# thunlp/OpenMatch

Measured on NVIDIA H100. Metric: queries/sec top-1000 over 8.8M x 768 corpus, higher is better.
Workload: dtype f16

## Files before the change

openmatch_b200/csrc/ptx.cuh:

```cuda
#pragma once
#include <cuda_runtime.h>
#include <cuda_bf16.h>
#include <stdint.h>

#ifndef OM_WAIT_TIMEOUT_CYCLES
#define OM_WAIT_TIMEOUT_CYCLES (1000000000ll)
#endif

namespace om {

static __device__ unsigned int om_dev_fault;

__device__ __forceinline__ uint32_t smem_u32(const void* p) {
  return static_cast<uint32_t>(__cvta_generic_to_shared(p));
}

__device__ __forceinline__ void mbar_init(uint64_t* bar, uint32_t count) {
  asm volatile("mbarrier.init.shared::cta.b64 [%0], %1;" ::"r"(smem_u32(bar)), "r"(count) : "memory");
}
__device__ __forceinline__ void fence_barrier_init() {
  asm volatile("fence.mbarrier_init.release.cluster;" ::: "memory");
}
__device__ __forceinline__ void fence_proxy_async_smem() {
  asm volatile("fence.proxy.async.shared::cta;" ::: "memory");
}
__device__ __forceinline__ void fence_proxy_async_global() {
  asm volatile("fence.proxy.async.global;" ::: "memory");
}
__device__ __forceinline__ void mbar_arrive_expect_tx(uint64_t* bar, uint32_t bytes) {
  asm volatile("mbarrier.arrive.expect_tx.shared::cta.b64 _, [%0], %1;" ::"r"(smem_u32(bar)), "r"(bytes)
               : "memory");
}
__device__ __forceinline__ void mbar_arrive(uint64_t* bar) {
  asm volatile("mbarrier.arrive.shared::cta.b64 _, [%0];" ::"r"(smem_u32(bar)) : "memory");
}
__device__ __forceinline__ bool mbar_try_wait(uint64_t* bar, uint32_t parity) {
  uint32_t done;
  asm volatile(
      "{\n\t"
      ".reg .pred P;\n\t"
      "mbarrier.try_wait.parity.shared::cta.b64 P, [%1], %2;\n\t"
      "selp.u32 %0, 1, 0, P;\n\t"
      "}\n"
      : "=r"(done)
      : "r"(smem_u32(bar)), "r"(parity)
      : "memory");
  return done != 0;
}
static __device__ __noinline__ void mbar_wait_slow(uint64_t* bar, uint32_t parity, uint32_t site) {
  const long long t0 = clock64();
  uint32_t spins = 0;
  while (!mbar_try_wait(bar, parity)) {
    if ((++spins & 1023u) != 0) continue;
    if (*reinterpret_cast<volatile unsigned int*>(&om_dev_fault) != 0u) return;
    if (clock64() - t0 > OM_WAIT_TIMEOUT_CYCLES) {
      atomicCAS(&om_dev_fault, 0u, (site << 16) | (blockIdx.x & 0xffffu) | 0x80000000u);
      return;
    }
  }
}
__device__ __forceinline__ void mbar_wait(uint64_t* bar, uint32_t parity, uint32_t site) {
  if (mbar_try_wait(bar, parity)) return;
  if (mbar_try_wait(bar, parity)) return;
  mbar_wait_slow(bar, parity, site);
}
__device__ __forceinline__ void mbar_wait_warp(uint64_t* bar, uint32_t parity, uint32_t site) {
  if ((threadIdx.x & 31u) == 0) {
    if (!mbar_try_wait(bar, parity)) {
      const long long t0 = clock64();
      uint32_t spins = 0;
      while (!mbar_try_wait(bar, parity)) {
        __nanosleep(64);
        if ((++spins & 1023u) != 0) continue;
        if (*reinterpret_cast<volatile unsigned int*>(&om_dev_fault) != 0u) break;
        if (clock64() - t0 > OM_WAIT_TIMEOUT_CYCLES) {
          atomicCAS(&om_dev_fault, 0u, (site << 16) | (blockIdx.x & 0xffffu) | 0x80000000u);
          break;
        }
      }
    }
  }
  __syncwarp();
}
static inline unsigned int read_clear_dev_fault() {
  unsigned int v = 0, z = 0;
  if (cudaMemcpyFromSymbol(&v, om_dev_fault, sizeof(v)) != cudaSuccess) return 0xffffffffu;
  if (v) cudaMemcpyToSymbol(om_dev_fault, &z, sizeof(z));
  return v;
}

__device__ __forceinline__ void tma_prefetch_desc(const void* tmap) {
  asm volatile("prefetch.tensormap [%0];" ::"l"(reinterpret_cast<uint64_t>(tmap)) : "memory");
}
__device__ __forceinline__ void tma_load_2d(void* smem_dst, const void* tmap, uint64_t* bar, int32_t c0,
                                            int32_t c1) {
  asm volatile(
      "cp.async.bulk.tensor.2d.shared::cluster.global.tile.mbarrier::complete_tx::bytes"
      " [%0], [%1, {%3, %4}], [%2];"
      ::"r"(smem_u32(smem_dst)), "l"(reinterpret_cast<uint64_t>(tmap)), "r"(smem_u32(bar)), "r"(c0), "r"(c1)
      : "memory");
}
__device__ __forceinline__ void tma_prefetch_l2_2d(const void* tmap, int32_t c0, int32_t c1) {
  asm volatile("cp.async.bulk.prefetch.tensor.2d.L2.global.tile [%0, {%1, %2}];" ::"l"(reinterpret_cast<uint64_t>(tmap)),
               "r"(c0), "r"(c1)
               : "memory");
}
__device__ __forceinline__ void tma_store_2d(const void* tmap, const void* smem_src, int32_t c0, int32_t c1) {
  asm volatile("cp.async.bulk.tensor.2d.global.shared::cta.tile.bulk_group [%0, {%2, %3}], [%1];" ::"l"(
                   reinterpret_cast<uint64_t>(tmap)),
               "r"(smem_u32(smem_src)), "r"(c0), "r"(c1)
               : "memory");
}
__device__ __forceinline__ void bulk_commit_group() { asm volatile("cp.async.bulk.commit_group;" ::: "memory"); }
__device__ __forceinline__ void bulk_wait_group_read0() { asm volatile("cp.async.bulk.wait_group.read 0;" ::: "memory"); }
__device__ __forceinline__ void bulk_wait_group0() { asm volatile("cp.async.bulk.wait_group 0;" ::: "memory"); }

__device__ __forceinline__ void tma_load_2d_multicast(void* smem_dst, const void* tmap, uint64_t* bar, int32_t c0,
                                                      int32_t c1, uint16_t cta_mask) {
  asm volatile(
      "cp.async.bulk.tensor.2d.shared::cluster.global.tile.mbarrier::complete_tx::bytes.multicast::cluster"
      " [%0], [%1, {%3, %4}], [%2], %5;"
      ::"r"(smem_u32(smem_dst)), "l"(reinterpret_cast<uint64_t>(tmap)), "r"(smem_u32(bar)), "r"(c0), "r"(c1),
      "h"(cta_mask)
      : "memory");
}

__device__ __forceinline__ uint32_t cluster_ctarank() {
  uint32_t r;
  asm volatile("mov.u32 %0, %%cluster_ctarank;" : "=r"(r));
  return r;
}
__device__ __forceinline__ uint32_t cluster_id_x() {
  uint32_t r;
  asm volatile("mov.u32 %0, %%clusterid.x;" : "=r"(r));
  return r;
}
__device__ __forceinline__ uint32_t cluster_count_x() {
  uint32_t r;
  asm volatile("mov.u32 %0, %%nclusterid.x;" : "=r"(r));
  return r;
}
__device__ __forceinline__ void cluster_sync_all() {
  asm volatile("barrier.cluster.arrive.release.aligned;\n\tbarrier.cluster.wait.acquire.aligned;" ::: "memory");
}
__device__ __forceinline__ void mbar_arrive_remote(uint64_t* bar, uint32_t rank) {
  asm volatile(
      "{\n\t.reg .b32 ra;\n\t"
      "mapa.shared::cluster.u32 ra, %0, %1;\n\t"
      "mbarrier.arrive.shared::cluster.b64 _, [ra];\n\t}\n"
      ::"r"(smem_u32(bar)), "r"(rank)
      : "memory");
}

__device__ __forceinline__ void wgmma_fence() { asm volatile("wgmma.fence.sync.aligned;" ::: "memory"); }
__device__ __forceinline__ void wgmma_commit() { asm volatile("wgmma.commit_group.sync.aligned;" ::: "memory"); }
template <int N>
__device__ __forceinline__ void wgmma_wait() {
  asm volatile("wgmma.wait_group.sync.aligned %0;" ::"n"(N) : "memory");
}
template <int R>
__device__ __forceinline__ void wgmma_fence_regs(float (&d)[R]) {
#pragma unroll
  for (int i = 0; i < R; ++i) asm volatile("" : "+f"(d[i])::"memory");
}

__host__ __device__ constexpr uint64_t wgmma_desc_base(uint32_t lbo_bytes, uint32_t sbo_bytes) {
  return (static_cast<uint64_t>((lbo_bytes >> 4) & 0x3fffu) << 16) |
         (static_cast<uint64_t>((sbo_bytes >> 4) & 0x3fffu) << 32) | (1ull << 62);
}
__device__ __forceinline__ uint64_t wgmma_desc(uint32_t smem_addr, uint64_t base) {
  return base | static_cast<uint64_t>((smem_addr & 0x3ffffu) >> 4);
}
constexpr uint64_t kDescKMajorSW128 = wgmma_desc_base(16, 1024);

template <int TA, int TB>
__device__ __forceinline__ void wgmma_m64n128k16_bf16(float (&d)[64], uint64_t a_desc, uint64_t b_desc, uint32_t accumulate) {
  asm volatile(
      "{\n\t.reg .pred p;\n\tsetp.ne.b32 p, %66, 0;\n\t"
      "wgmma.mma_async.sync.aligned.m64n128k16.f32.bf16.bf16 {%0, %1, %2, %3, %4, %5, %6, %7, %8, %9, %10, %11, %12, %13, %14, %15, %16, %17, %18, %19, %20, %21, %22, %23, %24, %25, %26, %27, %28, %29, %30, %31, %32, %33, %34, %35, %36, %37, %38, %39, %40, %41, %42, %43, %44, %45, %46, %47, %48, %49, %50, %51, %52, %53, %54, %55, %56, %57, %58, %59, %60, %61, %62, %63}, %64, %65, p, 1, 1, %67, %68;\n\t}\n"
      : "+f"(d[0]), "+f"(d[1]), "+f"(d[2]), "+f"(d[3]), "+f"(d[4]), "+f"(d[5]), "+f"(d[6]), "+f"(d[7]), "+f"(d[8]), "+f"(d[9]), "+f"(d[10]), "+f"(d[11]), "+f"(d[12]), "+f"(d[13]), "+f"(d[14]), "+f"(d[15]), "+f"(d[16]), "+f"(d[17]), "+f"(d[18]), "+f"(d[19]), "+f"(d[20]), "+f"(d[21]), "+f"(d[22]), "+f"(d[23]), "+f"(d[24]), "+f"(d[25]), "+f"(d[26]), "+f"(d[27]), "+f"(d[28]), "+f"(d[29]), "+f"(d[30]), "+f"(d[31]), "+f"(d[32]), "+f"(d[33]), "+f"(d[34]), "+f"(d[35]), "+f"(d[36]), "+f"(d[37]), "+f"(d[38]), "+f"(d[39]), "+f"(d[40]), "+f"(d[41]), "+f"(d[42]), "+f"(d[43]), "+f"(d[44]), "+f"(d[45]), "+f"(d[46]), "+f"(d[47]), "+f"(d[48]), "+f"(d[49]), "+f"(d[50]), "+f"(d[51]), "+f"(d[52]), "+f"(d[53]), "+f"(d[54]), "+f"(d[55]), "+f"(d[56]), "+f"(d[57]), "+f"(d[58]), "+f"(d[59]), "+f"(d[60]), "+f"(d[61]), "+f"(d[62]), "+f"(d[63])
      : "l"(a_desc), "l"(b_desc), "r"(accumulate), "n"(TA), "n"(TB));
}
template <int TA, int TB>
__device__ __forceinline__ void wgmma_m64n128k16_f16(float (&d)[64], uint64_t a_desc, uint64_t b_desc, uint32_t accumulate) {
  asm volatile(
      "{\n\t.reg .pred p;\n\tsetp.ne.b32 p, %66, 0;\n\t"
      "wgmma.mma_async.sync.aligned.m64n128k16.f32.f16.f16 {%0, %1, %2, %3, %4, %5, %6, %7, %8, %9, %10, %11, %12, %13, %14, %15, %16, %17, %18, %19, %20, %21, %22, %23, %24, %25, %26, %27, %28, %29, %30, %31, %32, %33, %34, %35, %36, %37, %38, %39, %40, %41, %42, %43, %44, %45, %46, %47, %48, %49, %50, %51, %52, %53, %54, %55, %56, %57, %58, %59, %60, %61, %62, %63}, %64, %65, p, 1, 1, %67, %68;\n\t}\n"
      : "+f"(d[0]), "+f"(d[1]), "+f"(d[2]), "+f"(d[3]), "+f"(d[4]), "+f"(d[5]), "+f"(d[6]), "+f"(d[7]), "+f"(d[8]), "+f"(d[9]), "+f"(d[10]), "+f"(d[11]), "+f"(d[12]), "+f"(d[13]), "+f"(d[14]), "+f"(d[15]), "+f"(d[16]), "+f"(d[17]), "+f"(d[18]), "+f"(d[19]), "+f"(d[20]), "+f"(d[21]), "+f"(d[22]), "+f"(d[23]), "+f"(d[24]), "+f"(d[25]), "+f"(d[26]), "+f"(d[27]), "+f"(d[28]), "+f"(d[29]), "+f"(d[30]), "+f"(d[31]), "+f"(d[32]), "+f"(d[33]), "+f"(d[34]), "+f"(d[35]), "+f"(d[36]), "+f"(d[37]), "+f"(d[38]), "+f"(d[39]), "+f"(d[40]), "+f"(d[41]), "+f"(d[42]), "+f"(d[43]), "+f"(d[44]), "+f"(d[45]), "+f"(d[46]), "+f"(d[47]), "+f"(d[48]), "+f"(d[49]), "+f"(d[50]), "+f"(d[51]), "+f"(d[52]), "+f"(d[53]), "+f"(d[54]), "+f"(d[55]), "+f"(d[56]), "+f"(d[57]), "+f"(d[58]), "+f"(d[59]), "+f"(d[60]), "+f"(d[61]), "+f"(d[62]), "+f"(d[63])
      : "l"(a_desc), "l"(b_desc), "r"(accumulate), "n"(TA), "n"(TB));
}
template <int TA, int TB>
__device__ __forceinline__ void wgmma_m64n256k16_f16(float (&d)[128], uint64_t a_desc, uint64_t b_desc, uint32_t accumulate) {
  asm volatile(
      "{\n\t.reg .pred p;\n\tsetp.ne.b32 p, %130, 0;\n\t"
      "wgmma.mma_async.sync.aligned.m64n256k16.f32.f16.f16 {%0, %1, %2, %3, %4, %5, %6, %7, %8, %9, %10, %11, %12, %13, %14, %15, %16, %17, %18, %19, %20, %21, %22, %23, %24, %25, %26, %27, %28, %29, %30, %31, %32, %33, %34, %35, %36, %37, %38, %39, %40, %41, %42, %43, %44, %45, %46, %47, %48, %49, %50, %51, %52, %53, %54, %55, %56, %57, %58, %59, %60, %61, %62, %63, %64, %65, %66, %67, %68, %69, %70, %71, %72, %73, %74, %75, %76, %77, %78, %79, %80, %81, %82, %83, %84, %85, %86, %87, %88, %89, %90, %91, %92, %93, %94, %95, %96, %97, %98, %99, %100, %101, %102, %103, %104, %105, %106, %107, %108, %109, %110, %111, %112, %113, %114, %115, %116, %117, %118, %119, %120, %121, %122, %123, %124, %125, %126, %127}, %128, %129, p, 1, 1, %131, %132;\n\t}\n"
      : "+f"(d[0]), "+f"(d[1]), "+f"(d[2]), "+f"(d[3]), "+f"(d[4]), "+f"(d[5]), "+f"(d[6]), "+f"(d[7]), "+f"(d[8]), "+f"(d[9]), "+f"(d[10]), "+f"(d[11]), "+f"(d[12]), "+f"(d[13]), "+f"(d[14]), "+f"(d[15]), "+f"(d[16]), "+f"(d[17]), "+f"(d[18]), "+f"(d[19]), "+f"(d[20]), "+f"(d[21]), "+f"(d[22]), "+f"(d[23]), "+f"(d[24]), "+f"(d[25]), "+f"(d[26]), "+f"(d[27]), "+f"(d[28]), "+f"(d[29]), "+f"(d[30]), "+f"(d[31]), "+f"(d[32]), "+f"(d[33]), "+f"(d[34]), "+f"(d[35]), "+f"(d[36]), "+f"(d[37]), "+f"(d[38]), "+f"(d[39]), "+f"(d[40]), "+f"(d[41]), "+f"(d[42]), "+f"(d[43]), "+f"(d[44]), "+f"(d[45]), "+f"(d[46]), "+f"(d[47]), "+f"(d[48]), "+f"(d[49]), "+f"(d[50]), "+f"(d[51]), "+f"(d[52]), "+f"(d[53]), "+f"(d[54]), "+f"(d[55]), "+f"(d[56]), "+f"(d[57]), "+f"(d[58]), "+f"(d[59]), "+f"(d[60]), "+f"(d[61]), "+f"(d[62]), "+f"(d[63]), "+f"(d[64]), "+f"(d[65]), "+f"(d[66]), "+f"(d[67]), "+f"(d[68]), "+f"(d[69]), "+f"(d[70]), "+f"(d[71]), "+f"(d[72]), "+f"(d[73]), "+f"(d[74]), "+f"(d[75]), "+f"(d[76]), "+f"(d[77]), "+f"(d[78]), "+f"(d[79]), "+f"(d[80]), "+f"(d[81]), "+f"(d[82]), "+f"(d[83]), "+f"(d[84]), "+f"(d[85]), "+f"(d[86]), "+f"(d[87]), "+f"(d[88]), "+f"(d[89]), "+f"(d[90]), "+f"(d[91]), "+f"(d[92]), "+f"(d[93]), "+f"(d[94]), "+f"(d[95]), "+f"(d[96]), "+f"(d[97]), "+f"(d[98]), "+f"(d[99]), "+f"(d[100]), "+f"(d[101]), "+f"(d[102]), "+f"(d[103]), "+f"(d[104]), "+f"(d[105]), "+f"(d[106]), "+f"(d[107]), "+f"(d[108]), "+f"(d[109]), "+f"(d[110]), "+f"(d[111]), "+f"(d[112]), "+f"(d[113]), "+f"(d[114]), "+f"(d[115]), "+f"(d[116]), "+f"(d[117]), "+f"(d[118]), "+f"(d[119]), "+f"(d[120]), "+f"(d[121]), "+f"(d[122]), "+f"(d[123]), "+f"(d[124]), "+f"(d[125]), "+f"(d[126]), "+f"(d[127])
      : "l"(a_desc), "l"(b_desc), "r"(accumulate), "n"(TA), "n"(TB));
}

template <int N>
__device__ __forceinline__ void setmaxnreg_dec() {
  asm volatile("setmaxnreg.dec.sync.aligned.u32 %0;" ::"n"(N));
}
template <int N>
__device__ __forceinline__ void setmaxnreg_inc() {
  asm volatile("setmaxnreg.inc.sync.aligned.u32 %0;" ::"n"(N));
}
__device__ __forceinline__ void wgmma_m64n64k16_bf16_rs(float (&d)[32], const uint32_t (&a)[4], uint64_t b_desc, uint32_t accumulate) {
  asm volatile(
      "{\n\t.reg .pred p;\n\tsetp.ne.b32 p, %37, 0;\n\t"
      "wgmma.mma_async.sync.aligned.m64n64k16.f32.bf16.bf16 {%0, %1, %2, %3, %4, %5, %6, %7, %8, %9, %10, %11, %12, %13, %14, %15, %16, %17, %18, %19, %20, %21, %22, %23, %24, %25, %26, %27, %28, %29, %30, %31}, {%32, %33, %34, %35}, %36, p, 1, 1, 0;\n\t}\n"
      : "+f"(d[0]), "+f"(d[1]), "+f"(d[2]), "+f"(d[3]), "+f"(d[4]), "+f"(d[5]), "+f"(d[6]), "+f"(d[7]), "+f"(d[8]), "+f"(d[9]), "+f"(d[10]), "+f"(d[11]), "+f"(d[12]), "+f"(d[13]), "+f"(d[14]), "+f"(d[15]), "+f"(d[16]), "+f"(d[17]), "+f"(d[18]), "+f"(d[19]), "+f"(d[20]), "+f"(d[21]), "+f"(d[22]), "+f"(d[23]), "+f"(d[24]), "+f"(d[25]), "+f"(d[26]), "+f"(d[27]), "+f"(d[28]), "+f"(d[29]), "+f"(d[30]), "+f"(d[31])
      : "r"(a[0]), "r"(a[1]), "r"(a[2]), "r"(a[3]), "l"(b_desc), "r"(accumulate));
}
__device__ __forceinline__ void wgmma_m64n32k16_bf16_rs(float (&d)[16], const uint32_t (&a)[4], uint64_t b_desc, uint32_t accumulate) {
  asm volatile(
      "{\n\t.reg .pred p;\n\tsetp.ne.b32 p, %21, 0;\n\t"
      "wgmma.mma_async.sync.aligned.m64n32k16.f32.bf16.bf16 {%0, %1, %2, %3, %4, %5, %6, %7, %8, %9, %10, %11, %12, %13, %14, %15}, {%16, %17, %18, %19}, %20, p, 1, 1, 0;\n\t}\n"
      : "+f"(d[0]), "+f"(d[1]), "+f"(d[2]), "+f"(d[3]), "+f"(d[4]), "+f"(d[5]), "+f"(d[6]), "+f"(d[7]), "+f"(d[8]), "+f"(d[9]), "+f"(d[10]), "+f"(d[11]), "+f"(d[12]), "+f"(d[13]), "+f"(d[14]), "+f"(d[15])
      : "r"(a[0]), "r"(a[1]), "r"(a[2]), "r"(a[3]), "l"(b_desc), "r"(accumulate));
}

__device__ __forceinline__ uint32_t pack_bf16x2(float lo, float hi) {
  __nv_bfloat162 v = __floats2bfloat162_rn(lo, hi);
  return *reinterpret_cast<uint32_t*>(&v);
}
__device__ __forceinline__ float2 fma2(float2 a, float2 b, float2 c) { return make_float2(fmaf(a.x, b.x, c.x), fmaf(a.y, b.y, c.y)); }
__device__ __forceinline__ float2 mul2(float2 a, float2 b) { return make_float2(__fmul_rn(a.x, b.x), __fmul_rn(a.y, b.y)); }
__device__ __forceinline__ float2 splat2(float x) { return make_float2(x, x); }

__device__ __forceinline__ void named_bar_sync(uint32_t id, uint32_t nthreads) {
  asm volatile("bar.sync %0, %1;" ::"r"(id), "r"(nthreads) : "memory");
}

}
```

openmatch_b200/csrc/ring.cuh:

```cuda
#pragma once
#include "ptx.cuh"

namespace om {

template <int STAGES>
struct Ring {
  uint32_t stage = 0, phase = 0;
  __device__ __forceinline__ void advance() {
    if (++stage == STAGES) {
      stage = 0;
      phase ^= 1u;
    }
  }
};

__device__ __forceinline__ void ring_init(uint64_t* full, uint64_t* empty, int stages, uint32_t empty_arrivals) {
  for (int i = 0; i < stages; ++i) {
    mbar_init(&full[i], 1);
    mbar_init(&empty[i], empty_arrivals);
  }
}

template <int STAGES>
__device__ __forceinline__ void ring_wait_free(uint64_t* empty, const Ring<STAGES>& r, uint32_t site) {
  mbar_wait(&empty[r.stage], r.phase ^ 1u, site);
}

template <int STAGES>
__device__ __forceinline__ uint64_t* ring_acquire_tx(uint64_t* full, uint64_t* empty, const Ring<STAGES>& r,
                                                     uint32_t bytes, uint32_t site) {
  ring_wait_free(empty, r, site);
  mbar_arrive_expect_tx(&full[r.stage], bytes);
  return &full[r.stage];
}

template <int STAGES, class Issue, class Release>
__device__ __forceinline__ void ring_consume(uint64_t* full, Ring<STAGES>& r, int kb_begin, int kb_end, uint32_t site,
                                             Issue&& issue, Release&& release) {
  uint32_t prev_stage = 0;
  for (int kb = kb_begin; kb < kb_end; ++kb) {
    mbar_wait_warp(&full[r.stage], r.phase, site);
    wgmma_fence();
    issue(r.stage, kb != kb_begin ? 1u : 0u);
    wgmma_commit();
    if (kb != kb_begin) {
      wgmma_wait<1>();
      release(prev_stage);
    }
    prev_stage = r.stage;
    r.advance();
  }
  wgmma_wait<0>();
  if (kb_end > kb_begin) release(prev_stage);
}

}
```

openmatch_b200/csrc/scan_gemm.cuh:

```cuda
#pragma once
#include <cuda_fp16.h>

#include "scan_epilogue.cuh"

namespace om {

constexpr int kScanBlockN = 256;
constexpr int kScanStages = 3;
constexpr int kScanABytes = kBlockM * kBlockK * 2;
constexpr int kScanBBytes = kScanBlockN * kBlockK * 2;
constexpr int kScanStageBytes = kScanABytes + kScanBBytes;
constexpr int kScanConsumers = 256;
constexpr int kScanStash = 4;
constexpr int kScanStashOffset = kScanStages * kScanStageBytes;
constexpr int kScanStashBytes = 2 * 2 * kScanStash * kScanConsumers * 8;
constexpr int kScanBarOffset = kScanStashOffset + kScanStashBytes;
constexpr int kScanSmemBytes = kScanBarOffset + 2 * kScanStages * 8 + 1024;
static_assert(kScanSmemBytes <= 232448, "scan ring + stash exceed the 227 KB of shared memory an H100 block may use");

template <int H>
__device__ __forceinline__ float scan_pick(const float (&acc)[128], int i) {
  float a[32], b[16], c[8], d[4], e[2];
#pragma unroll
  for (int j = 0; j < 32; ++j) a[j] = (i & 1) ? acc[4 * j + 2 * H + 1] : acc[4 * j + 2 * H];
#pragma unroll
  for (int j = 0; j < 16; ++j) b[j] = (i & 2) ? a[2 * j + 1] : a[2 * j];
#pragma unroll
  for (int j = 0; j < 8; ++j) c[j] = (i & 4) ? b[2 * j + 1] : b[2 * j];
#pragma unroll
  for (int j = 0; j < 4; ++j) d[j] = (i & 8) ? c[2 * j + 1] : c[2 * j];
#pragma unroll
  for (int j = 0; j < 2; ++j) e[j] = (i & 16) ? d[2 * j + 1] : d[2 * j];
  return (i & 32) ? e[1] : e[0];
}

template <int H>
__device__ __forceinline__ int scan_filter_row(const float (&acc)[128], float t, int row, int lim, int q4, int col0,
                                               unsigned long long* stash, unsigned long long* cand, int* count,
                                               int* overflow, int C, uint32_t row_base) {
  float mx = acc[2 * H];
#pragma unroll
  for (int j = 0; j < 32; ++j) mx = fmaxf(mx, fmaxf(acc[4 * j + 2 * H], acc[4 * j + 2 * H + 1]));
  if (!(mx > t)) return 0;
  uint32_t lo = 0, hi = 0;
#pragma unroll
  for (int i = 0; i < 32; ++i) {
    lo |= (acc[4 * (i >> 1) + 2 * H + (i & 1)] > t ? 1u : 0u) << i;
    hi |= (acc[4 * (16 + (i >> 1)) + 2 * H + (i & 1)] > t ? 1u : 0u) << i;
  }
  unsigned long long mask = (static_cast<unsigned long long>(hi) << 32) | lo;
  if (lim < kScanBlockN) {
#pragma unroll 1
    for (int i = 0; i < 64; ++i)
      if (8 * (i >> 1) + 2 * q4 + (i & 1) >= lim) mask &= ~(1ull << i);
  }
  const int n = __popcll(mask);
  int pos = 0;
  if (n > kScanStash) {
    pos = atomicAdd(count + row, n - kScanStash);
    if (pos + (n - kScanStash) > C) *overflow = 1;
  }
  unsigned long long* mine = cand + static_cast<size_t>(row) * C;
  int idx = 0;
#pragma unroll 1
  while (mask) {
    const int i = __ffsll(static_cast<long long>(mask)) - 1;
    mask &= mask - 1;
    const unsigned long long key =
        make_key(scan_pick<H>(acc, i), row_base + static_cast<uint32_t>(col0 + 8 * (i >> 1) + 2 * q4 + (i & 1)));
    if (idx < kScanStash)
      stash[idx * kScanConsumers] = key;
    else if (pos + idx - kScanStash < C)
      mine[pos + idx - kScanStash] = key;
    ++idx;
  }
  return n < kScanStash ? n : kScanStash;
}

template <int CQ, int CX>
struct ScanCluster {
  static_assert((CQ == 2 || CQ == 4) && (CX == 1 || CX == 2), "scan cluster shapes: CQ in {2, 4}, CX in {1, 2}");
  static constexpr int kSize = CQ * CX;
  static constexpr int kShare = CQ + CX - 1;
  static constexpr int kQRows = kBlockM / CX;
  static constexpr int kXRows = kScanBlockN / CQ;
  static constexpr int kEmptyArrivals = kShare * (kScanConsumers / 32);
  __device__ static uint32_t peer_rank(uint32_t rank, int j) {
    const uint32_t a = rank % CQ, b = rank / CQ;
    if (j < CQ - 1) {
      const uint32_t o = static_cast<uint32_t>(j);
      return (o < a ? o : o + 1) + CQ * b;
    }
    const uint32_t o = static_cast<uint32_t>(j - (CQ - 1));
    return a + CQ * (o < b ? o : o + 1);
  }
  __device__ static uint16_t q_mask(uint32_t rank) {
    uint32_t m = 0;
#pragma unroll
    for (int b = 0; b < CX; ++b) m |= 1u << (rank % CQ + CQ * b);
    return static_cast<uint16_t>(m);
  }
  __device__ static uint16_t x_mask(uint32_t rank) {
    return static_cast<uint16_t>(((1u << CQ) - 1u) << (CQ * (rank / CQ)));
  }
};

template <int CQ, int CX>
__global__ void __launch_bounds__(kGemmProducerThreads + kScanConsumers, 1)
scan_wide_kernel(const __grid_constant__ CUtensorMap tmQ, const __grid_constant__ CUtensorMap tmX, int K,
                 const float* __restrict__ thr, unsigned long long* cand, int* count, int* overflow, int nq, int n_cols,
                 int C, uint32_t row_base) {
  using Cl = ScanCluster<CQ, CX>;
  extern __shared__ uint8_t smem_raw[];
  uint8_t* smem = reinterpret_cast<uint8_t*>((reinterpret_cast<uintptr_t>(smem_raw) + 1023) & ~uintptr_t(1023));
  unsigned long long* stash = reinterpret_cast<unsigned long long*>(smem + kScanStashOffset);
  uint64_t* full_bar = reinterpret_cast<uint64_t*>(smem + kScanBarOffset);
  uint64_t* empty_bar = full_bar + kScanStages;
  const uint32_t rank = cluster_ctarank();
  const int qa = static_cast<int>(rank % CQ), xb = static_cast<int>(rank / CQ);
  const int warp = __shfl_sync(0xffffffffu, static_cast<int>(threadIdx.x >> 5), 0);
  const int lane = static_cast<int>(threadIdx.x & 31);

  if (warp == 0 && lane == 0) {
    tma_prefetch_desc(&tmQ);
    tma_prefetch_desc(&tmX);
  }
  if (warp == 1 && lane == 0) {
    ring_init(full_bar, empty_bar, kScanStages, Cl::kEmptyArrivals);
    fence_barrier_init();
  }
  cluster_sync_all();

  const int qgroups = (nq + CQ * kBlockM - 1) / (CQ * kBlockM);
  const int num_tiles = qgroups * ((n_cols + CX * kScanBlockN - 1) / (CX * kScanBlockN));
  const int num_k = (K + kBlockK - 1) / kBlockK;

  if (warp < 4) {
    setmaxnreg_dec<40>();
    if (warp == 0 && lane == 0) {
      const uint16_t qmask = Cl::q_mask(rank), xmask = Cl::x_mask(rank);
      Ring<kScanStages> ring;
      for (int tile = static_cast<int>(cluster_id_x()); tile < num_tiles; tile += static_cast<int>(cluster_count_x())) {
        const int m_blk = (tile % qgroups) * CQ + qa;
        const int n_blk = (tile / qgroups) * CX + xb;
        for (int kb = 0; kb < num_k; ++kb) {
          uint64_t* bar = ring_acquire_tx(full_bar, empty_bar, ring, kScanStageBytes, 30);
          uint8_t* sa = smem + ring.stage * kScanStageBytes;
          if constexpr (CX == 1)
            tma_load_2d(sa, &tmQ, bar, kb * kBlockK, m_blk * kBlockM);
          else
            tma_load_2d_multicast(sa + xb * (Cl::kQRows * kBlockK * 2), &tmQ, bar, kb * kBlockK,
                                  m_blk * kBlockM + xb * Cl::kQRows, qmask);
          tma_load_2d_multicast(sa + kScanABytes + qa * (Cl::kXRows * kBlockK * 2), &tmX, bar, kb * kBlockK,
                                n_blk * kScanBlockN + qa * Cl::kXRows, xmask);
          ring.advance();
        }
      }
    }
  } else {
    setmaxnreg_inc<232>();
    const int et = static_cast<int>(threadIdx.x) - kGemmProducerThreads;
    const int wg = et >> 7;
    const int q4 = lane & 3;
    const int frow = 64 * wg + 16 * (warp & 3) + (lane >> 2);
    Ring<kScanStages> ring;
    int buf = 0;
    int p_n0 = 0, p_n1 = 0, p_excl0 = 0, p_excl1 = 0, p_pos0 = 0, p_pos1 = 0, p_row = 0, p_buf = 0;
    auto drain = [&]() {
      if (!__any_sync(0xffffffffu, (p_n0 | p_n1) != 0)) return;
      const int b0 = __shfl_sync(0xffffffffu, p_pos0, lane & ~3) + p_excl0;
      const int b1 = __shfl_sync(0xffffffffu, p_pos1, lane & ~3) + p_excl1;
      const unsigned long long* s = stash + p_buf * (2 * kScanStash * kScanConsumers) + et;
      unsigned long long* m0 = cand + static_cast<size_t>(p_row) * C;
      unsigned long long* m1 = cand + static_cast<size_t>(p_row + 8) * C;
      for (int j = 0; j < p_n0; ++j)
        if (b0 + j < C) m0[b0 + j] = s[j * kScanConsumers];
      for (int j = 0; j < p_n1; ++j)
        if (b1 + j < C) m1[b1 + j] = s[(kScanStash + j) * kScanConsumers];
      if ((p_n0 > 0 && b0 + p_n0 > C) || (p_n1 > 0 && b1 + p_n1 > C)) *overflow = 1;
      p_n0 = p_n1 = 0;
    };

    uint32_t peers[Cl::kShare - 1];
#pragma unroll
    for (int j = 0; j < Cl::kShare - 1; ++j) peers[j] = Cl::peer_rank(rank, j);
    auto release = [&](uint32_t s) {
      if (lane == 0) {
        mbar_arrive(&empty_bar[s]);
#pragma unroll
        for (int j = 0; j < Cl::kShare - 1; ++j) mbar_arrive_remote(&empty_bar[s], peers[j]);
      }
    };

    for (int tile = static_cast<int>(cluster_id_x()); tile < num_tiles; tile += static_cast<int>(cluster_count_x())) {
      const int m_blk = (tile % qgroups) * CQ + qa;
      const int n_blk = (tile / qgroups) * CX + xb;
      const int row0 = m_blk * kBlockM + frow, row1 = row0 + 8;
      const float inf = __int_as_float(0x7f800000);
      const float t0 = row0 < nq ? thr[row0] : inf, t1 = row1 < nq ? thr[row1] : inf;

      float acc[128];
#pragma unroll
      for (int i = 0; i < 128; ++i) acc[i] = 0.f;
      ring_consume(
          full_bar, ring, 0, num_k, 31,
          [&](uint32_t stage, uint32_t accumulate) {
            const uint32_t a_addr = smem_u32(smem + stage * kScanStageBytes) + wg * (64 * 128);
            const uint32_t b_addr = smem_u32(smem + stage * kScanStageBytes + kScanABytes);
#pragma unroll
            for (int k = 0; k < kBlockK / kWgmmaK; ++k)
              wgmma_m64n256k16_f16<0, 0>(acc, wgmma_desc(a_addr + k * 32, kDescKMajorSW128),
                                         wgmma_desc(b_addr + k * 32, kDescKMajorSW128), (accumulate | k) != 0 ? 1u : 0u);
          },
          release);
      wgmma_fence_regs(acc);

      drain();
      const int col0 = n_blk * kScanBlockN;
      const int lim = n_cols - col0;
      unsigned long long* sb = stash + buf * (2 * kScanStash * kScanConsumers) + et;
      const int k0 = scan_filter_row<0>(acc, t0, row0, lim, q4, col0, sb, cand, count, overflow, C, row_base);
      const int k1 = scan_filter_row<1>(acc, t1, row1, lim, q4, col0, sb + kScanStash * kScanConsumers, cand, count,
                                        overflow, C, row_base);
      if (__any_sync(0xffffffffu, (k0 | k1) != 0)) {
        int x0 = k0, x1 = k1;
        int y0 = __shfl_up_sync(0xffffffffu, x0, 1, 4), y1 = __shfl_up_sync(0xffffffffu, x1, 1, 4);
        if (q4 >= 1) x0 += y0, x1 += y1;
        y0 = __shfl_up_sync(0xffffffffu, x0, 2, 4), y1 = __shfl_up_sync(0xffffffffu, x1, 2, 4);
        if (q4 >= 2) x0 += y0, x1 += y1;
        const int n0 = __shfl_sync(0xffffffffu, x0, lane | 3), n1 = __shfl_sync(0xffffffffu, x1, lane | 3);
        if (q4 == 0) {
          if (n0 > 0) p_pos0 = atomicAdd(count + row0, n0);
          if (n1 > 0) p_pos1 = atomicAdd(count + row1, n1);
        }
        p_n0 = k0;
        p_n1 = k1;
        p_excl0 = x0 - k0;
        p_excl1 = x1 - k1;
        p_row = row0;
        p_buf = buf;
        buf ^= 1;
      }
    }
    drain();
  }

  __syncthreads();
  cluster_sync_all();
}

template <int CQ, int CX>
static inline cudaError_t scan_wide_max_clusters(int num_sms, int* out) {
  static int max_clusters = -1;
  if (max_clusters < 0) {
    constexpr int kSize = ScanCluster<CQ, CX>::kSize;
    cudaError_t e =
        cudaFuncSetAttribute(scan_wide_kernel<CQ, CX>, cudaFuncAttributeMaxDynamicSharedMemorySize, kScanSmemBytes);
    if (e != cudaSuccess) return e;
    cudaLaunchConfig_t cfg = {};
    cfg.gridDim = dim3(kSize * (num_sms / kSize));
    cfg.blockDim = dim3(kGemmProducerThreads + kScanConsumers);
    cfg.dynamicSmemBytes = kScanSmemBytes;
    cudaLaunchAttribute attr[1];
    attr[0].id = cudaLaunchAttributeClusterDimension;
    attr[0].val.clusterDim = {static_cast<unsigned>(kSize), 1, 1};
    cfg.attrs = attr;
    cfg.numAttrs = 1;
    int n = 0;
    e = cudaOccupancyMaxActiveClusters(&n, scan_wide_kernel<CQ, CX>, &cfg);
    if (e != cudaSuccess) return e;
    max_clusters = n < num_sms / kSize ? n : num_sms / kSize;
  }
  *out = max_clusters;
  return cudaSuccess;
}

template <int CQ, int CX>
static inline cudaError_t launch_scan_wide(const __half* Q, int64_t ldq, const __half* X, int64_t ldx, int nq, int n_cols,
                                           int K, const float* thr, unsigned long long* cand, int* count, int* overflow,
                                           int C, uint32_t row_base, int num_sms, cudaStream_t stream) {
  using Cl = ScanCluster<CQ, CX>;
  CUtensorMap tmQ, tmX;
  if (make_tmap_bf16_2d(&tmQ, Q, (uint64_t)K, (uint64_t)nq, (uint64_t)ldq * 2, kBlockK, Cl::kQRows) != 0)
    return cudaErrorInvalidValue;
  if (make_tmap_bf16_2d(&tmX, X, (uint64_t)K, (uint64_t)n_cols, (uint64_t)ldx * 2, kBlockK, Cl::kXRows) != 0)
    return cudaErrorInvalidValue;
  int max_clusters = 0;
  cudaError_t e = scan_wide_max_clusters<CQ, CX>(num_sms, &max_clusters);
  if (e != cudaSuccess) return e;
  if (max_clusters < 1) return cudaErrorNotSupported;
  cudaLaunchConfig_t cfg = {};
  cfg.blockDim = dim3(kGemmProducerThreads + kScanConsumers);
  cfg.dynamicSmemBytes = kScanSmemBytes;
  cfg.stream = stream;
  cudaLaunchAttribute attr[1];
  attr[0].id = cudaLaunchAttributeClusterDimension;
  attr[0].val.clusterDim = {static_cast<unsigned>(Cl::kSize), 1, 1};
  cfg.attrs = attr;
  cfg.numAttrs = 1;
  const int qgroups = (nq + CQ * kBlockM - 1) / (CQ * kBlockM);
  const int64_t num_tiles = static_cast<int64_t>(qgroups) * ((n_cols + CX * kScanBlockN - 1) / (CX * kScanBlockN));
  const int clusters = num_tiles < max_clusters ? static_cast<int>(num_tiles) : max_clusters;
  cfg.gridDim = dim3(Cl::kSize * clusters);
  return cudaLaunchKernelEx(&cfg, scan_wide_kernel<CQ, CX>, tmQ, tmX, K, thr, cand, count, overflow, nq, n_cols, C,
                            row_base);
}

static inline cudaError_t launch_scan_cluster(int cq, int cx, const __half* Q, int64_t ldq, const __half* X, int64_t ldx,
                                              int nq, int n_cols, int K, const float* thr, unsigned long long* cand,
                                              int* count, int* overflow, int C, uint32_t row_base, int num_sms,
                                              cudaStream_t stream) {
  if (nq <= 0 || n_cols <= 0 || K <= 0) return cudaSuccess;
  if (cq == 2 && cx == 1)
    return launch_scan_wide<2, 1>(Q, ldq, X, ldx, nq, n_cols, K, thr, cand, count, overflow, C, row_base, num_sms, stream);
  if (cq == 4 && cx == 1)
    return launch_scan_wide<4, 1>(Q, ldq, X, ldx, nq, n_cols, K, thr, cand, count, overflow, C, row_base, num_sms, stream);
  if (cq == 2 && cx == 2)
    return launch_scan_wide<2, 2>(Q, ldq, X, ldx, nq, n_cols, K, thr, cand, count, overflow, C, row_base, num_sms, stream);
  if (cq == 4 && cx == 2)
    return launch_scan_wide<4, 2>(Q, ldq, X, ldx, nq, n_cols, K, thr, cand, count, overflow, C, row_base, num_sms, stream);
  return cudaErrorInvalidValue;
}

static inline cudaError_t scan_cluster_capacity(int cq, int cx, int num_sms, int* out) {
  *out = -1;
  if (cq == 2 && cx == 1) return scan_wide_max_clusters<2, 1>(num_sms, out);
  if (cq == 4 && cx == 1) return scan_wide_max_clusters<4, 1>(num_sms, out);
  if (cq == 2 && cx == 2) return scan_wide_max_clusters<2, 2>(num_sms, out);
  if (cq == 4 && cx == 2) return scan_wide_max_clusters<4, 2>(num_sms, out);
  return cudaSuccess;
}

}
```

Measured before the change: 37960.

## Stagger consumer warpgroups, peel first k-block, skip empty query tiles, deepen ring

Adds a peeled ring-consume loop in which the first k-block uses an init WGMMA variant with write-only accumulators, so the explicit zeroing of 128 accumulator registers is dropped. Warpgroup 1 waits on a named barrier until warpgroup 0 has issued its first MMA batch. This offsets the two consumer warpgroups so their filter/epilogue phases overlap the other group's tensor-core work. Tiles whose query block lies entirely past nq now only consume and release ring stages without computing. The ring also grows from 3 to 4 stages, which raises shared memory use and could limit occupancy or cluster fit.

```diff
diff --git a/openmatch_b200/csrc/ptx.cuh b/openmatch_b200/csrc/ptx.cuh
--- a/openmatch_b200/csrc/ptx.cuh
+++ b/openmatch_b200/csrc/ptx.cuh
@@ -198,6 +198,15 @@
       : "l"(a_desc), "l"(b_desc), "r"(accumulate), "n"(TA), "n"(TB));
 }
 
+template <int TA, int TB>
+__device__ __forceinline__ void wgmma_m64n256k16_f16_init(float (&d)[128], uint64_t a_desc, uint64_t b_desc) {
+  asm volatile(
+      "{\n\t.reg .pred p;\n\tsetp.ne.b32 p, %130, 0;\n\t"
+      "wgmma.mma_async.sync.aligned.m64n256k16.f32.f16.f16 {%0, %1, %2, %3, %4, %5, %6, %7, %8, %9, %10, %11, %12, %13, %14, %15, %16, %17, %18, %19, %20, %21, %22, %23, %24, %25, %26, %27, %28, %29, %30, %31, %32, %33, %34, %35, %36, %37, %38, %39, %40, %41, %42, %43, %44, %45, %46, %47, %48, %49, %50, %51, %52, %53, %54, %55, %56, %57, %58, %59, %60, %61, %62, %63, %64, %65, %66, %67, %68, %69, %70, %71, %72, %73, %74, %75, %76, %77, %78, %79, %80, %81, %82, %83, %84, %85, %86, %87, %88, %89, %90, %91, %92, %93, %94, %95, %96, %97, %98, %99, %100, %101, %102, %103, %104, %105, %106, %107, %108, %109, %110, %111, %112, %113, %114, %115, %116, %117, %118, %119, %120, %121, %122, %123, %124, %125, %126, %127}, %128, %129, p, 1, 1, %131, %132;\n\t}\n"
+      : "=f"(d[0]), "=f"(d[1]), "=f"(d[2]), "=f"(d[3]), "=f"(d[4]), "=f"(d[5]), "=f"(d[6]), "=f"(d[7]), "=f"(d[8]), "=f"(d[9]), "=f"(d[10]), "=f"(d[11]), "=f"(d[12]), "=f"(d[13]), "=f"(d[14]), "=f"(d[15]), "=f"(d[16]), "=f"(d[17]), "=f"(d[18]), "=f"(d[19]), "=f"(d[20]), "=f"(d[21]), "=f"(d[22]), "=f"(d[23]), "=f"(d[24]), "=f"(d[25]), "=f"(d[26]), "=f"(d[27]), "=f"(d[28]), "=f"(d[29]), "=f"(d[30]), "=f"(d[31]), "=f"(d[32]), "=f"(d[33]), "=f"(d[34]), "=f"(d[35]), "=f"(d[36]), "=f"(d[37]), "=f"(d[38]), "=f"(d[39]), "=f"(d[40]), "=f"(d[41]), "=f"(d[42]), "=f"(d[43]), "=f"(d[44]), "=f"(d[45]), "=f"(d[46]), "=f"(d[47]), "=f"(d[48]), "=f"(d[49]), "=f"(d[50]), "=f"(d[51]), "=f"(d[52]), "=f"(d[53]), "=f"(d[54]), "=f"(d[55]), "=f"(d[56]), "=f"(d[57]), "=f"(d[58]), "=f"(d[59]), "=f"(d[60]), "=f"(d[61]), "=f"(d[62]), "=f"(d[63]), "=f"(d[64]), "=f"(d[65]), "=f"(d[66]), "=f"(d[67]), "=f"(d[68]), "=f"(d[69]), "=f"(d[70]), "=f"(d[71]), "=f"(d[72]), "=f"(d[73]), "=f"(d[74]), "=f"(d[75]), "=f"(d[76]), "=f"(d[77]), "=f"(d[78]), "=f"(d[79]), "=f"(d[80]), "=f"(d[81]), "=f"(d[82]), "=f"(d[83]), "=f"(d[84]), "=f"(d[85]), "=f"(d[86]), "=f"(d[87]), "=f"(d[88]), "=f"(d[89]), "=f"(d[90]), "=f"(d[91]), "=f"(d[92]), "=f"(d[93]), "=f"(d[94]), "=f"(d[95]), "=f"(d[96]), "=f"(d[97]), "=f"(d[98]), "=f"(d[99]), "=f"(d[100]), "=f"(d[101]), "=f"(d[102]), "=f"(d[103]), "=f"(d[104]), "=f"(d[105]), "=f"(d[106]), "=f"(d[107]), "=f"(d[108]), "=f"(d[109]), "=f"(d[110]), "=f"(d[111]), "=f"(d[112]), "=f"(d[113]), "=f"(d[114]), "=f"(d[115]), "=f"(d[116]), "=f"(d[117]), "=f"(d[118]), "=f"(d[119]), "=f"(d[120]), "=f"(d[121]), "=f"(d[122]), "=f"(d[123]), "=f"(d[124]), "=f"(d[125]), "=f"(d[126]), "=f"(d[127])
+      : "l"(a_desc), "l"(b_desc), "r"(0u), "n"(TA), "n"(TB));
+}
+
 template <int N>
 __device__ __forceinline__ void setmaxnreg_dec() {
   asm volatile("setmaxnreg.dec.sync.aligned.u32 %0;" ::"n"(N));
@@ -232,5 +241,8 @@
 __device__ __forceinline__ void named_bar_sync(uint32_t id, uint32_t nthreads) {
   asm volatile("bar.sync %0, %1;" ::"r"(id), "r"(nthreads) : "memory");
 }
-
-}
+__device__ __forceinline__ void named_bar_arrive(uint32_t id, uint32_t nthreads) {
+  asm volatile("bar.arrive %0, %1;" ::"r"(id), "r"(nthreads) : "memory");
+}
+
+}
diff --git a/openmatch_b200/csrc/ring.cuh b/openmatch_b200/csrc/ring.cuh
--- a/openmatch_b200/csrc/ring.cuh
+++ b/openmatch_b200/csrc/ring.cuh
@@ -54,4 +54,31 @@
   if (kb_end > kb_begin) release(prev_stage);
 }
 
+template <int STAGES, class Issue, class Release>
+__device__ __forceinline__ void ring_consume_peeled(uint64_t* full, Ring<STAGES>& r, int kb_begin, int kb_end,
+                                                    uint32_t site, Issue&& issue, Release&& release) {
+  if (kb_end <= kb_begin) {
+    wgmma_wait<0>();
+    return;
+  }
+  mbar_wait_warp(&full[r.stage], r.phase, site);
+  wgmma_fence();
+  issue(r.stage, 0u);
+  wgmma_commit();
+  uint32_t prev_stage = r.stage;
+  r.advance();
+  for (int kb = kb_begin + 1; kb < kb_end; ++kb) {
+    mbar_wait_warp(&full[r.stage], r.phase, site);
+    wgmma_fence();
+    issue(r.stage, 1u);
+    wgmma_commit();
+    wgmma_wait<1>();
+    release(prev_stage);
+    prev_stage = r.stage;
+    r.advance();
+  }
+  wgmma_wait<0>();
+  release(prev_stage);
 }
+
+}
diff --git a/openmatch_b200/csrc/scan_gemm.cuh b/openmatch_b200/csrc/scan_gemm.cuh
--- a/openmatch_b200/csrc/scan_gemm.cuh
+++ b/openmatch_b200/csrc/scan_gemm.cuh
@@ -6,7 +6,7 @@
 namespace om {
 
 constexpr int kScanBlockN = 256;
-constexpr int kScanStages = 3;
+constexpr int kScanStages = 4;
 constexpr int kScanABytes = kBlockM * kBlockK * 2;
 constexpr int kScanBBytes = kScanBlockN * kBlockK * 2;
 constexpr int kScanStageBytes = kScanABytes + kScanBBytes;
@@ -192,25 +192,43 @@
       }
     };
 
+    bool lead = wg == 0;
+    auto stagger = [&]() {
+      if (lead) {
+        named_bar_arrive(1, kScanConsumers);
+        lead = false;
+      }
+    };
+    if (wg == 1) named_bar_sync(1, kScanConsumers);
+
     for (int tile = static_cast<int>(cluster_id_x()); tile < num_tiles; tile += static_cast<int>(cluster_count_x())) {
       const int m_blk = (tile % qgroups) * CQ + qa;
       const int n_blk = (tile / qgroups) * CX + xb;
+      if (m_blk * kBlockM >= nq) {
+        ring_consume_peeled(full_bar, ring, 0, num_k, 32, [&](uint32_t, uint32_t) { stagger(); }, release);
+        drain();
+        continue;
+      }
       const int row0 = m_blk * kBlockM + frow, row1 = row0 + 8;
       const float inf = __int_as_float(0x7f800000);
       const float t0 = row0 < nq ? thr[row0] : inf, t1 = row1 < nq ? thr[row1] : inf;
 
       float acc[128];
-#pragma unroll
-      for (int i = 0; i < 128; ++i) acc[i] = 0.f;
-      ring_consume(
+      ring_consume_peeled(
           full_bar, ring, 0, num_k, 31,
           [&](uint32_t stage, uint32_t accumulate) {
             const uint32_t a_addr = smem_u32(smem + stage * kScanStageBytes) + wg * (64 * 128);
             const uint32_t b_addr = smem_u32(smem + stage * kScanStageBytes + kScanABytes);
 #pragma unroll
-            for (int k = 0; k < kBlockK / kWgmmaK; ++k)
-              wgmma_m64n256k16_f16<0, 0>(acc, wgmma_desc(a_addr + k * 32, kDescKMajorSW128),
-                                         wgmma_desc(b_addr + k * 32, kDescKMajorSW128), (accumulate | k) != 0 ? 1u : 0u);
+            for (int k = 0; k < kBlockK / kWgmmaK; ++k) {
+              const uint64_t da = wgmma_desc(a_addr + k * 32, kDescKMajorSW128);
+              const uint64_t db = wgmma_desc(b_addr + k * 32, kDescKMajorSW128);
+              if (k == 0 && !accumulate)
+                wgmma_m64n256k16_f16_init<0, 0>(acc, da, db);
+              else
+                wgmma_m64n256k16_f16<0, 0>(acc, da, db, 1u);
+            }
+            stagger();
           },
           release);
       wgmma_fence_regs(acc);
@@ -242,6 +260,7 @@
         buf ^= 1;
       }
     }
+    stagger();
     drain();
   }
 
```

After: 38750, median of 6. 2.1% higher.
